# lcicek/Critic-VAE

Hardware: AMD Instinct MI355X
Metric: VAE train-step images/sec on 64x64x3 frames (higher is better)
Workload: dtype f32

## Files before the change

critic-vae_amd/csrc/api.hip:

```cpp
#include "common.h"
#include "../../include/cvae.h"
#include <stdarg.h>
#include <stdio.h>
#include <stdlib.h>
#include <string.h>
#include <cmath>
#include <string>
#include <vector>

static thread_local char g_err[512] = "";
void cvae_set_error(const char* fmt, ...) {
    va_list ap;
    va_start(ap, fmt);
    vsnprintf(g_err, sizeof(g_err), fmt, ap);
    va_end(ap);
}

static constexpr int PROBE_IDS = 32, PROBE_CAP = 128;
struct ProbeSlot { hipEvent_t e0[PROBE_CAP], e1[PROBE_CAP]; int n = 0; bool made = false; };
struct ProbeState { uint32_t mask = 0; ProbeSlot slot[PROBE_IDS]; };
static thread_local ProbeSlot* g_probe_cur = nullptr;
void cvae_probe_begin(hipStream_t st) {
    ProbeSlot* p = g_probe_cur;
    if (p && p->n < PROBE_CAP) (void)hipEventRecord(p->e0[p->n], st);
// ... 22 lines not shown
}

int persistent_grid(int wgs_per_cu, int num_items) {
    static const int maxwg = [] { const char* e = getenv("CVAE_PERSIST_MAXWG"); const int n = e ? atoi(e) : 0; return n > 0 ? n : 0; }();
    int G = wgs_per_cu * cvae_num_cus();
    if (maxwg > 0 && G > maxwg) G = maxwg;
    G -= G % 8;
    if (G < 8) G = 8;
    return G < num_items ? G : num_items;
}
extern "C" int32_t cvae_conv_route(int32_t precision, int32_t width, int32_t layer, int32_t dgrad, int64_t batch) {
    if ((width != 64 && width != 128) || layer < 0 || layer > 3 || precision < 0 || precision > 3 || batch < 1 || batch > 0x7fffffffLL) return CVAE_EINVAL;
    if (layer == 0 && (precision != 1 || dgrad != 0)) return CVAE_EINVAL;
    return conv_route(precision, layer, width, dgrad != 0, batch).family;
}

struct ParamEntry { std::string name; int64_t offset, numel; };

struct WsLayout {
    int64_t y[4], a[4], coef[4], bnpart[4];
    int64_t zcat, h, o[4];
    int64_t dout4, d_o[4], d_h, d_zcat, d_a[4], d_y[4];
    int64_t wc[3];
    int64_t xp;
    int64_t wpack;
    int64_t ms, scratch_w, scratch, total;
};

struct cvae_handle_s {
    cvae_config cfg;
    std::vector<ParamEntry> params;
    int64_t param_total;
    int K;
    int enc_w[4], enc_b[4], enc_g[4], enc_be[4], fc_w, fc_b, dec_w[5], dec_b[5], di_w, di_b;
    hipStream_t side = nullptr;
    hipEvent_t ev_ready[8] = {}, ev_side = nullptr;
    bool streams_ready = false;
    const void* xp_ws = nullptr;
    int xp_B = 0;
    struct { int pass = 0, next = 0, B = 0; const void* ws = nullptr; const double* rec = nullptr; } sync;
    ProbeState probe;
};

struct ProbeArm {
    ProbeArm(cvae_handle_s* h, int kind, int layer) {
        const int id = kind * 9 + layer;
// ... 23 lines not shown
    auto take = [&](int64_t n) { int64_t o = off; off += align_up(n, 64); return o; };
    const bool b16 = h->cfg.precision == 1;
    auto act = [&](int64_t elems) { return take(b16 ? (elems + 1) / 2 : elems); };
    for (int l = 0; l < 4; ++l) {
        const int64_t H = layer_h(h, l), C = kLayers[l].cout;
        w.y[l] = act(B * H * H * C);
        w.a[l] = act(B * (H / 2) * (H / 2) * C);
        w.coef[l] = take(C * 4);
        w.bnpart[l] = take((int64_t)2 * bn_num_tiles(l, W, B) * C);
        w.d_y[l] = l == 0 ? -1 : act(B * H * H * C);
        w.d_a[l] = act(B * (H / 2) * (H / 2) * C);
    }
    w.zcat = take((int64_t)B * 33);
    w.d_zcat = take((int64_t)B * 33);
    w.h = act((int64_t)B * h->K);
    w.d_h = act((int64_t)B * h->K);
    for (int i = 0; i < 4; ++i) {
        const int64_t H = layer_h(h, 4 + i), C = kLayers[4 + i].cout;
        w.o[i] = act(B * H * H * C);
        w.d_o[i] = act(B * H * H * C);
    }
    w.dout4 = take(b16 ? 0 : (int64_t)B * 3 * W * W);
    for (int i = 0; i < 3; ++i) w.wc[i] = take(conv_up_wc_floats(5 + i));
    w.xp = take(b16 ? (int64_t)B * W * W * 2 : 0);
    w.wpack = take(h->cfg.precision != 0 ? conv_bf16_pack_floats(h->cfg.precision >= 2 ? 3 : 1) : 0);
    w.ms = take(msssim_ws_floats(W, B));
    int64_t sc = 0, scw = 0;
    auto mx = [&](int64_t v) { if (v > sc) sc = v; };
    for (int l = 1; l <= 4; ++l) { if (wgrad_ws_floats(l, W, B) > scw) scw = wgrad_ws_floats(l, W, B);
        if (h->cfg.precision == 1 && conv_bf16_supported(l, W) && wgrad_bf16_ws_floats(l, W, B) > scw) scw = wgrad_bf16_ws_floats(l, W, B);
        if (h->cfg.precision >= 2 && conv_bf16_supported(l, W) && wgrad_split_ws_floats(l, W, B) > scw) scw = wgrad_split_ws_floats(l, W, B);
        mx(conv_fwd_ws_floats(l, W, B)); mx(conv_dgrad_ws_floats(l, W, B)); }
    for (int l = 5; l <= 7; ++l) { if (conv_up_wgrad_ws_floats(l, W, B) > scw) scw = conv_up_wgrad_ws_floats(l, W, B); mx(conv_up_ws_floats(l, W, B)); }
    if (e1_wgrad_ws_floats(W, B) > scw) scw = e1_wgrad_ws_floats(W, B);
    w.scratch_w = take(scw);
    mx(scw + 36 * 128 * 64);
    mx(d4_bwd_ws_floats(W, B));
    for (int l = 0; l < 4; ++l) { mx(bn_bwd_ws_floats(l, W, B)); mx(bn_fwd_ws_floats(l, W)); }
    mx(fc_ws_floats(W, B));
    mx(colsum_ws_floats(0, 256));
    w.scratch = take(sc);
    w.total = off;
    return w;
}

static void add_param(cvae_handle_s* h, int* idx, const char* name, int64_t numel) {
// ... 43 lines not shown
    }
    delete h;
}

int64_t cvae_param_total(cvae_handle h) { return h->param_total; }
int32_t cvae_param_count(cvae_handle h) { return (int32_t)h->params.size(); }
const char* cvae_param_name(cvae_handle h, int32_t i) { return h->params[i].name.c_str(); }
int64_t cvae_param_offset(cvae_handle h, int32_t i) { return h->params[i].offset; }
int64_t cvae_param_numel(cvae_handle h, int32_t i) { return h->params[i].numel; }
int64_t cvae_workspace_bytes(cvae_handle h, int32_t batch) { return carve(h, batch).total * 4; }
int64_t cvae_bn_state_floats(cvae_handle) { return 2 * 480; }

int64_t cvae_ws_offset(cvae_handle h, int32_t batch, const char* name) {
    const WsLayout w = carve(h, batch);
    char nm[32];
    for (int l = 0; l < 4; ++l) {
        snprintf(nm, sizeof nm, "y%d", l); if (!strcmp(name, nm)) return w.y[l];
        snprintf(nm, sizeof nm, "a%d", l); if (!strcmp(name, nm)) return w.a[l];
        snprintf(nm, sizeof nm, "d_y%d", l); if (!strcmp(name, nm)) return w.d_y[l];
        snprintf(nm, sizeof nm, "d_a%d", l); if (!strcmp(name, nm)) return w.d_a[l];
        snprintf(nm, sizeof nm, "coef%d", l); if (!strcmp(name, nm)) return w.coef[l];
        snprintf(nm, sizeof nm, "o%d", l); if (!strcmp(name, nm)) return w.o[l];
        snprintf(nm, sizeof nm, "d_o%d", l); if (!strcmp(name, nm)) return w.d_o[l];
    }
    if (!strcmp(name, "zcat")) return w.zcat;
    if (!strcmp(name, "d_zcat")) return w.d_zcat;
    if (!strcmp(name, "h")) return w.h;
    if (!strcmp(name, "d_h")) return w.d_h;
    if (!strcmp(name, "dout4")) return w.dout4;
    if (!strcmp(name, "scratch")) return w.scratch;
    if (!strcmp(name, "ms")) return w.ms;
    if (!strcmp(name, "xp")) return h->cfg.precision == 1 ? w.xp : -1;
    return -1;
}

static const int kBnOff[4] = {0, 32, 96, 224};
static const int64_t kSyncOff[9] = {0, 97, 289, 673, 1441, 1452, 1964, 2220, 2348};
static const int64_t kSyncCnt[9] = {97, 192, 384, 768, 11, 512, 256, 128, 64};
static const int64_t kSyncCount = 96;
static_assert(2348 + 64 == CVAE_SYNC_DOUBLES, "sync record size");
int cvae_decode(cvae_handle h, int32_t B, const float* zcat, const float* params, float* recon, void* wsv, void* stream);
int cvae_backward_phases(cvae_handle h, int32_t B, const float* x, const float* pred, const float* eps, const float* params,
                         const float* logvar, const float* recon, const float* d_recon, const float* d_mu,
                         const float* d_logvar, void* wsv, float* grads, int32_t phase_mask, void* stream);

#define P_(idx) (params + h->params[(idx)].offset)
// ... 228 lines not shown
        return 0;
    }
    int join() {
        if (!overlap) return 0;
        HIPRC(hipEventRecord(h->ev_side, h->side));
        HIPRC(hipStreamWaitEvent(st, h->ev_side, 0));
        return 0;
    }
    int decoder() {
        { ProbeArm pa(h, 1, 8);
          RC(launch_d4_bwd(W, B, ws + w.o[3], d_recon, recon, P_(h->dec_w[4]), ws + w.dout4, ws + w.d_o[3],
                           G_(h->dec_w[4]), G_(h->dec_b[4]), sc, st, io_bf16(h))); }
        for (int i = 3; i >= 0; --i) {
            const int l = 4 + i;
            const float* in = i == 0 ? ws + w.h : ws + w.o[i - 1];
            RC(fork(3 - i));
            if (i == 0) {
                { ProbeArm pa(h, 2, l); RC(conv_wgrad(h, 4, B, in, ws + w.d_o[0], G_(h->dec_w[0]), G_(h->dec_b[0]), scw, sd)); }
                { ProbeArm pa(h, 1, l);
                  if (use_bf16(h, 4)) RC(launch_conv_dgrad_bf16(4, W, bf16_mode(h), B, ws + w.d_o[0], ws + w.wpack, ws + w.d_h, ws + w.scratch, st));
                  else RC(launch_conv_dgrad(l, W, B, ws + w.d_o[0], P_(h->dec_w[0]), nullptr, ws + w.d_h, ws + w.scratch, st)); }
            } else {
                { ProbeArm pa(h, 2, l);
                  RC(launch_conv_up_wgrad(l, W, B, in, ws + w.d_o[i], G_(h->dec_w[i]), G_(h->dec_b[i]), scw, sd, use_bf16_wgrad(h, l))); }
                { ProbeArm pa(h, 1, l);
                  if (use_bf16(h, l)) RC(launch_conv_up_dgrad_bf16(l, W, bf16_mode(h), B, ws + w.d_o[i], ws + w.wpack, ws + w.o[i - 1], ws + w.d_o[i - 1], st));
                  else RC(launch_conv_up_dgrad(l, W, B, ws + w.d_o[i], ws + w.wc[i - 1], ws + w.o[i - 1], ws + w.d_o[i - 1], sc, st)); }
            }
        }
        RC(launch_decin_bwd(W, B, ws + w.zcat, ws + w.d_h, P_(h->di_w), G_(h->di_w), G_(h->di_b), ws + w.d_zcat, sc, st, io_bf16(h)));
        return join();
    }
    int fc() {
        return launch_fc_bwd(W, B, ws + w.a[3], P_(h->fc_w), ws + w.d_zcat, eps, logvar, d_mu, d_logvar, G_(h->fc_w),
                             G_(h->fc_b), ws + w.d_a[3], sc, st, io_bf16(h));
    }
    int bn(int l, int stage, double* rec, const double* count) {
        ProbeArm pa(h, 3, l);
        return launch_bn_pool_act_bwd(l, W, B, ws + w.y[l], ws + w.a[l], ws + w.d_a[l], ws + w.coef[l], P_(h->enc_g[l]),
                                      l == 0 ? nullptr : ws + w.d_y[l], G_(h->enc_g[l]), G_(h->enc_be[l]), nullptr, sc, st, io_bf16(h),
                                      stage, rec, count);
    }
    int block_grads(int l) {
        RC(fork(7 - l));
        if (l == 0) {
            const float* fu[7] = {ws + w.y[0], ws + w.a[0], ws + w.d_a[0], ws + w.coef[0], bn_bwd_bcoef(0, W, B, sc),
                                  P_(h->enc_w[0]), P_(h->enc_b[0])};
// ... 818 lines not shown
```

critic-vae_amd/csrc/bn.hip:

```cpp
#include "common.h"

struct BnGeom { int C, H, act; };
static inline BnGeom bn_geom(int layer, int width) {
    const int s = width / 64;
    return BnGeom{kLayers[layer].cout, kLayers[layer].h * s, layer == 3 ? 1 : 0};
}
static inline void part_geom(int layer, int H, int* imgs, int* pxPerImg, int* tilesPerImg) {
    if (layer == 0) { *imgs = 1; *pxPerImg = 512; *tilesPerImg = (H / 16) * (H / 32); return; }
    const TileGeom t = tile_geom(H);
    *imgs = t.IMGS; *pxPerImg = t.PX_PER_IMG; *tilesPerImg = t.TILES_PER_IMG;
}
int bn_num_tiles(int layer, int width, int B) {
    const BnGeom g = bn_geom(layer, width);
    int imgs, ppi, tpi;
    part_geom(layer, g.H, &imgs, &ppi, &tpi);
    return cdiv(B, imgs) * tpi;
}

__global__ __launch_bounds__(256) void bn_fwd_reduce_kernel(const float* __restrict__ part, int numTiles, int C, int B,
                                                            int imgsPerTile, int pxPerImg, int tilesPerImg,
                                                            double* __restrict__ mid, int tilesPerBlk) {
    __shared__ double red[3][8][32];
    const int cl = threadIdx.x & 31, rg = threadIdx.x >> 5, c = blockIdx.x * 32 + cl;
    const int t0 = blockIdx.y * tilesPerBlk;
    int t1 = t0 + tilesPerBlk; if (t1 > numTiles) t1 = numTiles;
    double S = 0.0, Q = 0.0, M = 0.0;
#pragma unroll 4
    for (int t = t0 + rg; t < t1; t += 8) {
        const int img0 = (t / tilesPerImg) * imgsPerTile;
        int ni = B - img0; if (ni > imgsPerTile) ni = imgsPerTile;
        const double n = (double)(ni * pxPerImg);
        const double s = (double)part[(size_t)t * C + c];
        S += s; Q += s * s / n; M += (double)part[((size_t)numTiles + t) * C + c];
    }
    red[0][rg][cl] = S; red[1][rg][cl] = Q; red[2][rg][cl] = M;
    __syncthreads();
    if (rg == 0) {
        for (int k = 1; k < 8; ++k) { S += red[0][k][cl]; Q += red[1][k][cl]; M += red[2][k][cl]; }
        double* o = mid + (size_t)blockIdx.y * 3 * C;
        o[c] = S; o[C + c] = Q; o[2 * C + c] = M;
    }
}

__device__ __forceinline__ void bn_fwd_coef(int c, double S, double Q, double M, double N, const float* __restrict__ gamma,
                                            const float* __restrict__ beta, float* __restrict__ run_mean,
                                            float* __restrict__ run_var, float* __restrict__ coef, int train) {
    float mean, var;
    if (train) {
        const double mu = S / N;
        double v = (M + Q - S * S / N) / N;
        if (v < 0.0) v = 0.0;
        mean = (float)mu; var = (float)v;
        const float uvar = (float)(v * N / (N - 1.0));
        {
#pragma clang fp contract(off)
            run_mean[c] = 0.9f * run_mean[c] + 0.1f * mean;
            run_var[c] = 0.9f * run_var[c] + 0.1f * uvar;
        }
    } else {
        mean = run_mean[c]; var = run_var[c];
    }
    const float invstd = 1.0f / sqrtf(var + 1e-5f);
    const float scale = gamma[c] * invstd;
    coef[c * 4 + 0] = scale;
    coef[c * 4 + 1] = beta[c] - mean * scale;
    coef[c * 4 + 2] = mean;
    coef[c * 4 + 3] = invstd;
}

struct BnSums { double S, Q, M; };
__device__ __forceinline__ BnSums bn_fwd_merge(const double* __restrict__ mid, int RA, int C, int c, int r) {
    BnSums s{0.0, 0.0, 0.0};
    if (r < RA) { s.S = mid[(size_t)r * 3 * C + c]; s.Q = mid[(size_t)r * 3 * C + C + c]; s.M = mid[(size_t)r * 3 * C + 2 * C + c]; }
#pragma unroll
    for (int o = 16; o > 0; o >>= 1) { s.S += __shfl_xor(s.S, o, 64); s.Q += __shfl_xor(s.Q, o, 64); s.M += __shfl_xor(s.M, o, 64); }
    return s;
}

__global__ __launch_bounds__(64) void bn_fwd_finalize_kernel(const double* __restrict__ mid, int RA, int C, double N,
                                                             const float* __restrict__ gamma, const float* __restrict__ beta,
                                                             float* __restrict__ run_mean, float* __restrict__ run_var,
                                                             float* __restrict__ coef, int train) {
    const int c = blockIdx.x * 2 + (threadIdx.x >> 5), r = threadIdx.x & 31;
    const BnSums s = bn_fwd_merge(mid, train ? RA : 0, C, c, r);
    if (r != 0) return;
    bn_fwd_coef(c, s.S, s.Q, s.M, N, gamma, beta, run_mean, run_var, coef, train);
}

__global__ __launch_bounds__(64) void bn_fwd_record_kernel(const double* __restrict__ mid, int RA, int C, double* __restrict__ rec,
                                                           double* __restrict__ count, double images) {
    const int c = blockIdx.x * 2 + (threadIdx.x >> 5), r = threadIdx.x & 31;
    const BnSums s = bn_fwd_merge(mid, RA, C, c, r);
    if (r != 0) return;
    rec[c] = s.S; rec[C + c] = s.Q; rec[2 * C + c] = s.M;
    if (count && c == 0) *count = images;
}

__global__ __launch_bounds__(64) void bn_fwd_finish_kernel(const double* __restrict__ rec, const double* __restrict__ count, int C, int H,
                                                           const float* __restrict__ gamma, const float* __restrict__ beta,
                                                           float* __restrict__ run_mean, float* __restrict__ run_var,
                                                           float* __restrict__ coef) {
    const int c = blockIdx.x * 64 + threadIdx.x;
    if (c >= C) return;
    const double N = count[0] * H * H;
    bn_fwd_coef(c, rec[c], rec[C + c], rec[2 * C + c], N, gamma, beta, run_mean, run_var, coef, 1);
}

__device__ __forceinline__ float act_fwd(float v, int act) { return act ? tanhf(v) : fmaxf(v, 0.f); }
__device__ __forceinline__ float act_bwd_from_out(float a, int act) { return act ? (1.f - a * a) : (a > 0.f ? 1.f : 0.f); }
// ... 168 lines not shown
#pragma unroll
                for (int p = 0; p < 4; ++p) yy[p] = A::ld(y, base + window_px(p, H, C) + c);
                int pos;
                const float ym = window_argmax(yy, coef[c * 4], coef[c * 4 + 1], &pos);
                s2[e] += ((float)av[e] > 0.f ? (float)gv[e] : 0.f) * ((ym - coef[c * 4 + 2]) * coef[c * 4 + 3]);
            }
        }
    }
#pragma unroll
    for (int e = 0; e < V; ++e) { red[0][threadIdx.x][e] = s1[e]; red[1][threadIdx.x][e] = s2[e]; }
    __syncthreads();
    if (sub == 0) {
        for (int k = 1; k < NSUB; ++k)
#pragma unroll
            for (int e = 0; e < V; ++e) { s1[e] += red[0][k * CV + cv][e]; s2[e] += red[1][k * CV + cv][e]; }
#pragma unroll
        for (int e = 0; e < V; ++e) {
            part[((size_t)blockIdx.x * 2) * C + cv * V + e] = s1[e];
            part[((size_t)blockIdx.x * 2 + 1) * C + cv * V + e] = s2[e];
        }
    }
}

template <bool REC>
__global__ __launch_bounds__(256) void bn_bwd_finalize_kernel(const float* __restrict__ rows, int R, int64_t stride, int C, float invN,
                                                              float* __restrict__ dgamma, float* __restrict__ dbeta, float* __restrict__ bcoef,
                                                              double* __restrict__ rec) {
    const int c = blockIdx.x * 16 + (threadIdx.x >> 4), q = threadIdx.x & 15;
    float s1 = 0.f, s2 = 0.f;
    if (c < C)
        for (int r = q; r < R; r += 16) { s1 += rows[(size_t)r * stride + c]; s2 += rows[(size_t)r * stride + C + c]; }
#pragma unroll
    for (int o = 8; o > 0; o >>= 1) { s1 += __shfl_xor(s1, o, 64); s2 += __shfl_xor(s2, o, 64); }
    if (c < C && q == 0) {
        dgamma[c] = s2; dbeta[c] = s1;
        if (REC) { rec[c] = (double)s1; rec[C + c] = (double)s2; }
        else { bcoef[c * 2] = s1 * invN; bcoef[c * 2 + 1] = s2 * invN; }
    }
}

__global__ __launch_bounds__(256) void bn_bwd_finish_kernel(const double* __restrict__ rec, const double* __restrict__ count, int C, int H,
                                                            float* __restrict__ bcoef) {
    const int c = blockIdx.x * 256 + threadIdx.x;
    if (c >= C) return;
    const float invN = (float)(1.0 / (double)(float)(count[0] * H * H));
    bcoef[c * 2] = (float)rec[c] * invN;
    bcoef[c * 2 + 1] = (float)rec[C + c] * invN;
}

static constexpr int BN_RA = 32;
int64_t bn_fwd_ws_floats(int layer, int width) { (void)width; return (int64_t)2 * BN_RA * 3 * kLayers[layer].cout; }

static int bn_fwd_reduce(int layer, int width, int B, const float* bnpart, float* ws, hipStream_t st, int tilesPerPartial, int* RA_out) {
    const BnGeom g = bn_geom(layer, width);
    int imgs, ppi, tpi;
    part_geom(layer, g.H, &imgs, &ppi, &tpi);
    int numTiles = cdiv(B, imgs) * tpi;
    if (tilesPerPartial > 1) {
        const int T = tilesPerPartial;
        numTiles = cdiv(numTiles, T);
        if (tpi >= T) { ppi *= T; tpi /= T; }
        else if (tpi > 1) { imgs = T / tpi; ppi *= tpi; tpi = 1; }
        else imgs *= T;
    }
    double* mid = reinterpret_cast<double*>(ws);
    const int tpb = cdiv(numTiles, BN_RA);
    const int RA = cdiv(numTiles, tpb);
    hipLaunchKernelGGL(bn_fwd_reduce_kernel, dim3(g.C / 32, RA), dim3(256), 0, st, bnpart, numTiles, g.C, B, imgs,
                       ppi, tpi, mid, tpb);
    CVAE_CHECK_LAUNCH();
    *RA_out = RA;
    return 0;
}

int launch_bn_fwd_finalize(int layer, int width, int B, const float* bnpart, const float* gamma, const float* beta,
                           float* run_mean, float* run_var, float* coef, float* ws, int train, hipStream_t st, int tilesPerPartial) {
    const BnGeom g = bn_geom(layer, width);
    double* mid = reinterpret_cast<double*>(ws);
    int RA = 0;
    if (train) { int rc = bn_fwd_reduce(layer, width, B, bnpart, ws, st, tilesPerPartial, &RA); if (rc) return rc; }
    hipLaunchKernelGGL(bn_fwd_finalize_kernel, dim3(g.C / 2), dim3(64), 0, st, mid, RA, g.C,
                       (double)B * g.H * g.H, gamma, beta, run_mean, run_var, coef, train);
    CVAE_CHECK_LAUNCH();
    return 0;
}

int launch_bn_fwd_record(int layer, int width, int B, const float* bnpart, float* ws, hipStream_t st, int tilesPerPartial,
                         double* rec, double* count) {
    const BnGeom g = bn_geom(layer, width);
    int RA = 0;
    { int rc = bn_fwd_reduce(layer, width, B, bnpart, ws, st, tilesPerPartial, &RA); if (rc) return rc; }
    hipLaunchKernelGGL(bn_fwd_record_kernel, dim3(g.C / 2), dim3(64), 0, st, reinterpret_cast<const double*>(ws), RA, g.C,
                       rec, count, (double)B);
    CVAE_CHECK_LAUNCH();
    return 0;
}

int launch_bn_fwd_finish(int layer, int width, const double* rec, const double* count, const float* gamma, const float* beta,
                         float* run_mean, float* run_var, float* coef, hipStream_t st) {
    const BnGeom g = bn_geom(layer, width);
    hipLaunchKernelGGL(bn_fwd_finish_kernel, dim3(cdiv(g.C, 64)), dim3(64), 0, st, rec, count, g.C, g.H, gamma, beta,
                       run_mean, run_var, coef);
    CVAE_CHECK_LAUNCH();
    return 0;
}
// ... 37 lines not shown
static BnBwdKernels bn_bwd_kernels() {
    if constexpr (ACT == 0) return {bn_bwd_stats_relu_kernel<AT>, bn_bwd_kernel<AT, 0, 1>};
    else return {bn_bwd_kernel<AT, ACT, 0>, bn_bwd_kernel<AT, ACT, 1>};
}

int launch_bn_pool_act_bwd(int layer, int width, int B, const float* y, const float* a, const float* da,
                           const float* coef, const float* gamma, float* dy, float* dgamma, float* dbeta,
                           float* dbias, float* ws, hipStream_t st, bool bf16io, int stage, double* rec, const double* count) {
    (void)gamma;
    const BnGeom g = bn_geom(layer, width);
    const int64_t totalPx = (int64_t)B * (g.H / 2) * (g.H / 2);
    const int nblk = bn_bwd_blocks(totalPx, g.C);
    const int64_t ppb = (totalPx + nblk - 1) / nblk;
    float* part = ws;
    float* bcoef = ws + (size_t)nblk * 2 * g.C;
    float* red = bcoef + 2 * g.C;
    float* crws = red + 2 * g.C;
    const float invN = 1.0f / (float)((double)B * g.H * g.H);
    const BnBwdKernels k = bf16io ? (g.act ? bn_bwd_kernels<__bf16, 1>() : bn_bwd_kernels<__bf16, 0>())
                                  : (g.act ? bn_bwd_kernels<float, 1>() : bn_bwd_kernels<float, 0>());
    if (stage != 2) {
        hipLaunchKernelGGL(k.stats, dim3(nblk), dim3(256), 0, st, y, a, da, coef, nullptr, nullptr, part, g.C, g.H, totalPx, ppb);
        CVAE_CHECK_LAUNCH();
        const float* rows; int R; int64_t rstride;
        { int rc = launch_col_reduce_partial(part, nblk, 2 * g.C, 2 * g.C, crws, st, &rows, &R, &rstride); if (rc) return rc; }
        if (stage == 1) hipLaunchKernelGGL(bn_bwd_finalize_kernel<true>, dim3(cdiv(g.C, 16)), dim3(256), 0, st, rows, R, rstride, g.C, invN, dgamma, dbeta, nullptr, rec);
        else hipLaunchKernelGGL(bn_bwd_finalize_kernel<false>, dim3(cdiv(g.C, 16)), dim3(256), 0, st, rows, R, rstride, g.C, invN, dgamma, dbeta, bcoef, nullptr);
        CVAE_CHECK_LAUNCH();
        if (stage == 1) return 0;
    } else {
        hipLaunchKernelGGL(bn_bwd_finish_kernel, dim3(cdiv(g.C, 256)), dim3(256), 0, st, rec, count, g.C, g.H, bcoef);
        CVAE_CHECK_LAUNCH();
    }
    if (!dy) {
        if (dbias) { cvae_set_error("bn_bwd: dbias needs the apply pass (dy)"); return -2; }
        return 0;
    }
    cvae_probe_begin(st);
    hipLaunchKernelGGL(k.apply, dim3(nblk), dim3(256), 0, st, y, a, da, coef, bcoef, dy, part, g.C, g.H, totalPx, ppb);
    cvae_probe_end(st);
    CVAE_CHECK_LAUNCH();
    if (dbias) return launch_col_reduce(part, nblk, g.C, g.C, dbias, crws, st);
    return 0;
}
```

critic-vae_amd/csrc/common.h:

```cpp
#pragma once
#include <hip/hip_runtime.h>
#include <stdint.h>
#include <stddef.h>
#include <atomic>

typedef float f32x16 __attribute__((ext_vector_type(16)));
typedef float f32x4 __attribute__((ext_vector_type(4)));
typedef __bf16 bf16x8 __attribute__((ext_vector_type(8)));

typedef __bf16 bf16x4 __attribute__((ext_vector_type(4)));

template <typename AT> struct Act;
template <> struct Act<float> {
    static constexpr bool BF16 = false;
    static __device__ __forceinline__ float ld(const float* p, size_t i) { return p[i]; }
    static __device__ __forceinline__ void st(float* p, size_t i, float v) { p[i] = v; }
    static __device__ __forceinline__ f32x4 ld4(const float* p, size_t i) { return *reinterpret_cast<const f32x4*>(p + i); }
    static __device__ __forceinline__ void st4(float* p, size_t i, f32x4 v) { *reinterpret_cast<f32x4*>(p + i) = v; }
    template <int V> using Vec = float __attribute__((ext_vector_type(V)));
    template <int V> static __device__ __forceinline__ Vec<V> ldv(const float* p, size_t i) {
        static_assert(V == 1 || V == 4, "fp32 storage: scalar or float4 accesses");
        return *reinterpret_cast<const Vec<V>*>(p + i);
    }
    template <int V> static __device__ __forceinline__ void stv(float* p, size_t i, Vec<V> v) {
// ... 191 lines not shown
                  float* xp = nullptr);
int launch_e1_wgrad(int width, int B, const float* x, const float* dy, float* dw, float* dbias, float* ws,
                    hipStream_t st, bool bf16 = false, const float* const* fuse = nullptr,
                    const float* xp = nullptr);
const float* bn_bwd_bcoef(int layer, int width, int B, const float* ws);
int64_t e1_wgrad_ws_floats(int width, int B);
int launch_d4_fwd(int width, int B, const float* in, const float* w, const float* bias, float* recon,
                  hipStream_t st, bool bf16io = false);
int64_t d4_bwd_ws_floats(int width, int B);
int launch_d4_bwd(int width, int B, const float* o3, const float* d_recon, const float* recon,
                  const float* w, float* dout, float* d_o3, float* dw, float* db, float* ws,
                  hipStream_t st, bool bf16io = false);
int64_t conv_up_wc_floats(int layer);
int launch_collapse_w(int layer, const float* w, float* wc, hipStream_t st);
int launch_collapse_w3(const float* const w[3], float* const wc[3], hipStream_t st);
int64_t conv_up_ws_floats(int layer, int width, int B);
int launch_conv_up_fwd(int layer, int width, int B, const float* in, const float* wc, const float* bias,
                       float* out, float* ws, hipStream_t st);
int launch_conv_up_dgrad(int layer, int width, int B, const float* dout, const float* wc, const float* aux,
                         float* din, float* ws, hipStream_t st);
int64_t conv_up_wgrad_ws_floats(int layer, int width, int B);
int launch_conv_up_wgrad(int layer, int width, int B, const float* in, const float* dout, float* dw,
                         float* dbias, float* ws, hipStream_t st, bool bf16 = false);
int launch_up_wgrad_bf16_main(int layer, int width, int B, const float* in, const float* dout, float* slab, int Smax, int* S_out, hipStream_t st,
                              int* plan = nullptr);
int conv_wgrad_bf16_plan(int layer, int width, int B, int plan[3]);
int conv_up_wgrad_bf16_plan(int layer, int width, int B, int plan[3]);
int bn_num_tiles(int layer, int width, int B);
int launch_bn_fwd_finalize(int layer, int width, int B, const float* bnpart, const float* gamma,
                           const float* beta, float* run_mean, float* run_var, float* coef,
                           float* ws, int train, hipStream_t st, int tilesPerPartial = 1);
int launch_bn_fwd_record(int layer, int width, int B, const float* bnpart, float* ws, hipStream_t st, int tilesPerPartial,
                         double* rec, double* count);
int launch_bn_fwd_finish(int layer, int width, const double* rec, const double* count, const float* gamma, const float* beta,
                         float* run_mean, float* run_var, float* coef, hipStream_t st);
int64_t bn_fwd_ws_floats(int layer, int width);
int launch_bn_pool_act_fwd(int layer, int width, int B, const float* y, const float* coef, float* a,
                           hipStream_t st, bool bf16io = false);
int64_t bn_bwd_ws_floats(int layer, int width, int B);
int launch_bn_pool_act_bwd(int layer, int width, int B, const float* y, const float* a,
                           const float* da, const float* coef, const float* gamma, float* dy,
                           float* dgamma, float* dbeta, float* dbias, float* ws, hipStream_t st, bool bf16io = false,
                           int stage = 0, double* rec = nullptr, const double* count = nullptr);
struct LatentPlan {
    int fc_fwd_gemm;
    int di_imgs, di_blocks;
// ... 116 lines not shown
```

critic-vae_amd/csrc/conv_up.hip:

```cpp
#include "common.h"

static constexpr int KC = 16, KCP = 17;

template <int HS>
struct UpTile {
    static constexpr int TW = HS < 32 ? HS : 32;
    static constexpr int TH = (128 / TW) < HS ? (128 / TW) : HS;
    static constexpr int IMGS = 128 / (TW * TH);
    static constexpr int HTW = TW + 2, HTH = TH + 2, HPI = HTW * HTH, HP = IMGS * HPI;
    static constexpr int PS = ((HP + 5) / 8) * 8 + 2;
    static constexpr int TILES_X = HS / TW, TILES_Y = HS / TH, TILES_PER_IMG = TILES_X * TILES_Y;
};

__device__ __forceinline__ int phase_lo(int ph, int a) { return ph == 0 ? (a == 0 ? 0 : a == 1 ? 2 : 4) : (a == 0 ? 0 : a == 1 ? 1 : 3); }
__device__ __forceinline__ int phase_hi(int ph, int a) { return ph == 0 ? (a == 0 ? 1 : a == 1 ? 3 : 4) : (a == 0 ? 0 : a == 1 ? 2 : 4); }
__device__ __forceinline__ int phase_of(int ph, int r) { return ph == 0 ? (r >> 1) : ((r + 1) >> 1); }

struct CollapseJobs { const float* w[3]; float* wc[3]; int n[3]; };
__global__ __launch_bounds__(256) void collapse_w_kernel(CollapseJobs jobs) {
    const float* __restrict__ w = jobs.w[blockIdx.z];
    float* __restrict__ wc = jobs.wc[blockIdx.z];
    const int n = jobs.n[blockIdx.z];
    const int i = blockIdx.x * 256 + threadIdx.x;
    if (i >= n) return;
    const int t = blockIdx.y, p = t / 9, a = (t % 9) / 3, b = t % 3, py = p >> 1, px = p & 1;
    float acc = 0.f;
    for (int r = phase_lo(py, a); r <= phase_hi(py, a); ++r)
        for (int s = phase_lo(px, b); s <= phase_hi(px, b); ++s) acc += w[(size_t)(r * 5 + s) * n + i];
    wc[(size_t)t * n + i] = acc;
}

__global__ __launch_bounds__(256) void expand_dw_kernel(const float* __restrict__ rows, int R, int64_t stride,
                                                        float* __restrict__ dw, int n, float* __restrict__ dbias,
                                                        int cout) {
    const int i = blockIdx.x * 256 + threadIdx.x;
    if (dbias != nullptr && blockIdx.x == 0 && blockIdx.y == 0 && (int)threadIdx.x < cout) {
        float b = 0.f;
        for (int q = 0; q < R; ++q) b += rows[(size_t)q * stride + (size_t)36 * n + threadIdx.x];
        dbias[threadIdx.x] = b;
    }
    if (i >= n) return;
    const int r = blockIdx.y / 5, s = blockIdx.y % 5;
    float acc = 0.f;
#pragma unroll
    for (int p = 0; p < 4; ++p) {
        const float* src = rows + (size_t)(p * 9 + phase_of(p >> 1, r) * 3 + phase_of(p & 1, s)) * n + i;
        float a = 0.f;
        for (int q = 0; q < R; ++q) a += src[(size_t)q * stride];
        acc += a;
    }
    dw[(size_t)blockIdx.y * n + i] = acc;
}

struct UpArgs {
    const float* in;
    const float* wc;
    const float* bias;
// ... 455 lines not shown

int launch_conv_up_dgrad(int layer, int width, int B, const float* dout, const float* wc, const float* aux, float* din,
                         float* ws, hipStream_t st) {
    if (width == 64) {
        switch (layer) {
            case 5: return run_up_dgrad<128, 64, 4, 64, UP_KS5>(B, dout, wc, aux, din, ws, st);
            case 6: return run_up_dgrad<64, 32, 8, 64, UP_KS6>(B, dout, wc, aux, din, ws, st);
            case 7: return run_up_dgrad<32, 32, 16, 32, 1>(B, dout, wc, aux, din, ws, st);
        }
    }
    if (width == 128) {
        switch (layer) {
            case 5: return run_up_dgrad<128, 64, 8, 64, UP_KS5>(B, dout, wc, aux, din, ws, st);
            case 6: return run_up_dgrad<64, 32, 16, 64, UP_KS6>(B, dout, wc, aux, din, ws, st);
            case 7: return run_up_dgrad<32, 32, 32, 32, 1>(B, dout, wc, aux, din, ws, st);
        }
    }
    cvae_set_error("conv_up_dgrad: unsupported layer %d at width %d", layer, width);
    return -2;
}

template <int CIN, int COUT, int HS>
static int run_up_wgrad(int B, const float* in, const float* dout, float* dw, float* dbias, float* ws, hipStream_t st,
                        int64_t* need, int bf16_layer = 0, int bf16_width = 64, int* plan = nullptr) {
    using T = UpTile64<HS>;
    const int numTiles = cdiv(B, T::IMGS) * T::TILES_PER_IMG;
    const int bps = (CIN / 32) * (COUT / 32);
    const int cus = cvae_num_cus();
    int Scap = cdiv(2 * cus, bps);
    if (Scap > numTiles) Scap = numTiles;
    int S = cdiv(cus, bps);
    if (S > numTiles) S = numTiles;
    const int tps = cdiv(numTiles, S);
    S = cdiv(numTiles, tps);
    const int64_t nc = (int64_t)36 * CIN * COUT, row = nc + COUT;
    if (plan) return launch_up_wgrad_bf16_main(bf16_layer, bf16_width, B, nullptr, nullptr, nullptr, Scap, &S, st, plan);
    if (need) { *need = (int64_t)(Scap + 17) * row; return 0; }
    if (bf16_layer) {
        int rc = launch_up_wgrad_bf16_main(bf16_layer, bf16_width, B, in, dout, ws, Scap, &S, st);
        if (rc) return rc;
    } else {
        UpWgradArgs a{in, dout, ws, B, numTiles, tps};
        cvae_probe_begin(st);
        hipLaunchKernelGGL((conv_up_wgrad_kernel<CIN, COUT, HS>), dim3(S, CIN / 32, COUT / 32), dim3(256), 0, st, a);
        cvae_probe_end(st);
        CVAE_CHECK_LAUNCH();
    }
    float* mid = ws + (size_t)S * row;
    float* red = mid + (size_t)16 * row;
    { int rc = launch_reduce_slabs(ws, red, row, S, row, st, mid); if (rc) return rc; }
    const float* rows = red;
    const int R = 1;
    static_assert(COUT <= 256, "expand_dw_kernel sums the bias gradient in one workgroup");
    hipLaunchKernelGGL(expand_dw_kernel, dim3(cdiv(CIN * COUT, 256), 25), dim3(256), 0, st, rows, R, row, dw, CIN * COUT, dbias, COUT);
    CVAE_CHECK_LAUNCH();
    return 0;
}

static int dispatch_up_wgrad(int layer, int width, int B, const float* in, const float* dout, float* dw, float* dbias,
                             float* ws, hipStream_t st, int64_t* need, bool bf16 = false, int* plan = nullptr) {
    if (width == 64) {
        switch (layer) {
            case 5: return run_up_wgrad<128, 64, 4>(B, in, dout, dw, dbias, ws, st, need, bf16 ? 5 : 0, 64, plan);
            case 6: return run_up_wgrad<64, 32, 8>(B, in, dout, dw, dbias, ws, st, need, bf16 ? 6 : 0, 64, plan);
            case 7: return run_up_wgrad<32, 32, 16>(B, in, dout, dw, dbias, ws, st, need, bf16 ? 7 : 0, 64, plan);
        }
    }
    if (width == 128) {
        switch (layer) {
            case 5: return run_up_wgrad<128, 64, 8>(B, in, dout, dw, dbias, ws, st, need, bf16 ? 5 : 0, 128, plan);
            case 6: return run_up_wgrad<64, 32, 16>(B, in, dout, dw, dbias, ws, st, need, bf16 ? 6 : 0, 128, plan);
            case 7: return run_up_wgrad<32, 32, 32>(B, in, dout, dw, dbias, ws, st, need, bf16 ? 7 : 0, 128, plan);
        }
    }
    cvae_set_error("conv_up_wgrad: unsupported layer %d at width %d", layer, width);
    return -2;
}
int64_t conv_up_wgrad_ws_floats(int layer, int width, int B) {
    int64_t need = 0;
    if (dispatch_up_wgrad(layer, width, B, nullptr, nullptr, nullptr, nullptr, nullptr, nullptr, &need)) return 0;
    return need;
}
int conv_up_wgrad_bf16_plan(int layer, int width, int B, int plan[3]) {
    return dispatch_up_wgrad(layer, width, B, nullptr, nullptr, nullptr, nullptr, nullptr, nullptr, nullptr, true, plan);
}
int launch_conv_up_wgrad(int layer, int width, int B, const float* in, const float* dout, float* dw, float* dbias,
                         float* ws, hipStream_t st, bool bf16) {
    return dispatch_up_wgrad(layer, width, B, in, dout, dw, dbias, ws, st, nullptr, bf16);
}
```

Baseline: 90490.

## Batch decoder expand_dw launches and fuse BN reduce/finalize into single kernels

Decoder up-conv wgrad now writes its reduced slab into dedicated workspace buffers, and one batched expand_dw launch covers all three layers, replacing three separate launches. BN forward statistics use a single 1024-thread kernel that reduces and finalizes when the tile count is small. BN backward in stage 0 skips the column-reduce pass and finalizes directly from the partials. The aim is to cut kernel launches and intermediate passes in a launch-bound train step. The cost is extra workspace and a batched expand that now runs only after the last wgrad has finished.

```diff
diff --git a/critic-vae_amd/csrc/api.hip b/critic-vae_amd/csrc/api.hip
--- a/critic-vae_amd/csrc/api.hip
+++ b/critic-vae_amd/csrc/api.hip
@@ -68,6 +68,7 @@
     int64_t zcat, h, o[4];
     int64_t dout4, d_o[4], d_h, d_zcat, d_a[4], d_y[4];
     int64_t wc[3];
+    int64_t up_red[3];
     int64_t xp;
     int64_t wpack;
     int64_t ms, scratch_w, scratch, total;
@@ -137,6 +138,7 @@
     }
     w.dout4 = take(b16 ? 0 : (int64_t)B * 3 * W * W);
     for (int i = 0; i < 3; ++i) w.wc[i] = take(conv_up_wc_floats(5 + i));
+    for (int i = 0; i < 3; ++i) w.up_red[i] = take(conv_up_red_floats(5 + i));
     w.xp = take(b16 ? (int64_t)B * W * W * 2 : 0);
     w.wpack = take(h->cfg.precision != 0 ? conv_bf16_pack_floats(h->cfg.precision >= 2 ? 3 : 1) : 0);
     w.ms = take(msssim_ws_floats(W, B));
@@ -226,6 +228,7 @@
         snprintf(nm, sizeof nm, "coef%d", l); if (!strcmp(name, nm)) return w.coef[l];
         snprintf(nm, sizeof nm, "o%d", l); if (!strcmp(name, nm)) return w.o[l];
         snprintf(nm, sizeof nm, "d_o%d", l); if (!strcmp(name, nm)) return w.d_o[l];
+        snprintf(nm, sizeof nm, "up_red%d", l); if (l < 3 && !strcmp(name, nm)) return w.up_red[l];
     }
     if (!strcmp(name, "zcat")) return w.zcat;
     if (!strcmp(name, "d_zcat")) return w.d_zcat;
@@ -500,7 +503,13 @@
                   else RC(launch_conv_dgrad(l, W, B, ws + w.d_o[0], P_(h->dec_w[0]), nullptr, ws + w.d_h, ws + w.scratch, st)); }
             } else {
                 { ProbeArm pa(h, 2, l);
-                  RC(launch_conv_up_wgrad(l, W, B, in, ws + w.d_o[i], G_(h->dec_w[i]), G_(h->dec_b[i]), scw, sd, use_bf16_wgrad(h, l))); }
+                  RC(launch_conv_up_wgrad_reduce(l, W, B, in, ws + w.d_o[i], ws + w.up_red[i - 1], scw, sd, use_bf16_wgrad(h, l))); }
+                if (i == 1) {
+                    const float* red[3] = {ws + w.up_red[0], ws + w.up_red[1], ws + w.up_red[2]};
+                    float* dw[3] = {G_(h->dec_w[1]), G_(h->dec_w[2]), G_(h->dec_w[3])};
+                    float* db[3] = {G_(h->dec_b[1]), G_(h->dec_b[2]), G_(h->dec_b[3])};
+                    RC(launch_expand_dw3(red, dw, db, sd));
+                }
                 { ProbeArm pa(h, 1, l);
                   if (use_bf16(h, l)) RC(launch_conv_up_dgrad_bf16(l, W, bf16_mode(h), B, ws + w.d_o[i], ws + w.wpack, ws + w.o[i - 1], ws + w.d_o[i - 1], st));
                   else RC(launch_conv_up_dgrad(l, W, B, ws + w.d_o[i], ws + w.wc[i - 1], ws + w.o[i - 1], ws + w.d_o[i - 1], sc, st)); }
diff --git a/critic-vae_amd/csrc/bn.hip b/critic-vae_amd/csrc/bn.hip
--- a/critic-vae_amd/csrc/bn.hip
+++ b/critic-vae_amd/csrc/bn.hip
@@ -15,6 +15,21 @@
     int imgs, ppi, tpi;
     part_geom(layer, g.H, &imgs, &ppi, &tpi);
     return cdiv(B, imgs) * tpi;
+}
+
+struct BnSums { double S, Q, M; };
+__device__ __forceinline__ BnSums bn_fwd_rows(const float* __restrict__ part, int numTiles, int C, int B, int imgsPerTile, int pxPerImg,
+                                              int tilesPerImg, int c, int t0, int t1, int rg) {
+    BnSums a{0.0, 0.0, 0.0};
+#pragma unroll 4
+    for (int t = t0 + rg; t < t1; t += 8) {
+        const int img0 = (t / tilesPerImg) * imgsPerTile;
+        int ni = B - img0; if (ni > imgsPerTile) ni = imgsPerTile;
+        const double n = (double)(ni * pxPerImg);
+        const double s = (double)part[(size_t)t * C + c];
+        a.S += s; a.Q += s * s / n; a.M += (double)part[((size_t)numTiles + t) * C + c];
+    }
+    return a;
 }
 
 __global__ __launch_bounds__(256) void bn_fwd_reduce_kernel(const float* __restrict__ part, int numTiles, int C, int B,
@@ -24,15 +39,8 @@
     const int cl = threadIdx.x & 31, rg = threadIdx.x >> 5, c = blockIdx.x * 32 + cl;
     const int t0 = blockIdx.y * tilesPerBlk;
     int t1 = t0 + tilesPerBlk; if (t1 > numTiles) t1 = numTiles;
-    double S = 0.0, Q = 0.0, M = 0.0;
-#pragma unroll 4
-    for (int t = t0 + rg; t < t1; t += 8) {
-        const int img0 = (t / tilesPerImg) * imgsPerTile;
-        int ni = B - img0; if (ni > imgsPerTile) ni = imgsPerTile;
-        const double n = (double)(ni * pxPerImg);
-        const double s = (double)part[(size_t)t * C + c];
-        S += s; Q += s * s / n; M += (double)part[((size_t)numTiles + t) * C + c];
-    }
+    const BnSums a = bn_fwd_rows(part, numTiles, C, B, imgsPerTile, pxPerImg, tilesPerImg, c, t0, t1, rg);
+    double S = a.S, Q = a.Q, M = a.M;
     red[0][rg][cl] = S; red[1][rg][cl] = Q; red[2][rg][cl] = M;
     __syncthreads();
     if (rg == 0) {
@@ -68,7 +76,6 @@
     coef[c * 4 + 3] = invstd;
 }
 
-struct BnSums { double S, Q, M; };
 __device__ __forceinline__ BnSums bn_fwd_merge(const double* __restrict__ mid, int RA, int C, int c, int r) {
     BnSums s{0.0, 0.0, 0.0};
     if (r < RA) { s.S = mid[(size_t)r * 3 * C + c]; s.Q = mid[(size_t)r * 3 * C + C + c]; s.M = mid[(size_t)r * 3 * C + 2 * C + c]; }
@@ -85,6 +92,30 @@
     const BnSums s = bn_fwd_merge(mid, train ? RA : 0, C, c, r);
     if (r != 0) return;
     bn_fwd_coef(c, s.S, s.Q, s.M, N, gamma, beta, run_mean, run_var, coef, train);
+}
+
+__global__ __launch_bounds__(1024) void bn_fwd_stats_kernel(const float* __restrict__ part, int numTiles, int C, int B,
+                                                            int imgsPerTile, int pxPerImg, int tilesPerImg, int tilesPerBlk, int RA,
+                                                            double N, const float* __restrict__ gamma, const float* __restrict__ beta,
+                                                            float* __restrict__ run_mean, float* __restrict__ run_var,
+                                                            float* __restrict__ coef) {
+    __shared__ double red[32][3][8][4];
+    const int cl = threadIdx.x & 3, rg = (threadIdx.x >> 2) & 7, ra = threadIdx.x >> 5;
+    const int t0 = ra * tilesPerBlk;
+    int t1 = t0 + tilesPerBlk; if (t1 > numTiles) t1 = numTiles;
+    BnSums a = bn_fwd_rows(part, numTiles, C, B, imgsPerTile, pxPerImg, tilesPerImg, blockIdx.x * 4 + cl, t0, t1, rg);
+    red[ra][0][rg][cl] = a.S; red[ra][1][rg][cl] = a.Q; red[ra][2][rg][cl] = a.M;
+    __syncthreads();
+    if (rg == 0) {
+        for (int k = 1; k < 8; ++k) { a.S += red[ra][0][k][cl]; a.Q += red[ra][1][k][cl]; a.M += red[ra][2][k][cl]; }
+        red[ra][0][0][cl] = a.S; red[ra][1][0][cl] = a.Q; red[ra][2][0][cl] = a.M;
+    }
+    __syncthreads();
+    if (threadIdx.x >= 128) return;
+    const int cm = threadIdx.x >> 5, r = threadIdx.x & 31;
+    const BnSums s = bn_fwd_merge(&red[0][0][0][0], RA, 32, cm, r);
+    if (r != 0) return;
+    bn_fwd_coef(blockIdx.x * 4 + cm, s.S, s.Q, s.M, N, gamma, beta, run_mean, run_var, coef, 1);
 }
 
 __global__ __launch_bounds__(64) void bn_fwd_record_kernel(const double* __restrict__ mid, int RA, int C, double* __restrict__ rec,
@@ -299,20 +330,54 @@
     }
 }
 
+struct BnBwdSums { float s1, s2; };
+__device__ __forceinline__ BnBwdSums bn_bwd_merge(const float* __restrict__ rows, int R, int64_t stride, int C, int c, int q, bool live) {
+    float s1 = 0.f, s2 = 0.f;
+    if (live)
+        for (int r = q; r < R; r += 16) { s1 += rows[(size_t)r * stride + c]; s2 += rows[(size_t)r * stride + C + c]; }
+#pragma unroll
+    for (int o = 8; o > 0; o >>= 1) { s1 += __shfl_xor(s1, o, 64); s2 += __shfl_xor(s2, o, 64); }
+    return BnBwdSums{s1, s2};
+}
+
 template <bool REC>
 __global__ __launch_bounds__(256) void bn_bwd_finalize_kernel(const float* __restrict__ rows, int R, int64_t stride, int C, float invN,
                                                               float* __restrict__ dgamma, float* __restrict__ dbeta, float* __restrict__ bcoef,
                                                               double* __restrict__ rec) {
     const int c = blockIdx.x * 16 + (threadIdx.x >> 4), q = threadIdx.x & 15;
-    float s1 = 0.f, s2 = 0.f;
-    if (c < C)
-        for (int r = q; r < R; r += 16) { s1 += rows[(size_t)r * stride + c]; s2 += rows[(size_t)r * stride + C + c]; }
-#pragma unroll
-    for (int o = 8; o > 0; o >>= 1) { s1 += __shfl_xor(s1, o, 64); s2 += __shfl_xor(s2, o, 64); }
+    const BnBwdSums s = bn_bwd_merge(rows, R, stride, C, c, q, c < C);
     if (c < C && q == 0) {
-        dgamma[c] = s2; dbeta[c] = s1;
-        if (REC) { rec[c] = (double)s1; rec[C + c] = (double)s2; }
-        else { bcoef[c * 2] = s1 * invN; bcoef[c * 2 + 1] = s2 * invN; }
+        dgamma[c] = s.s2; dbeta[c] = s.s1;
+        if (REC) { rec[c] = (double)s.s1; rec[C + c] = (double)s.s2; }
+        else { bcoef[c * 2] = s.s1 * invN; bcoef[c * 2 + 1] = s.s2 * invN; }
+    }
+}
+
+__global__ __launch_bounds__(1024) void bn_bwd_rows_finalize_kernel(const float* __restrict__ part, int R, int C, int rowsPerBlk, float invN,
+                                                                    float* __restrict__ dgamma, float* __restrict__ dbeta,
+                                                                    float* __restrict__ bcoef) {
+    __shared__ float red[32][2][8][4];
+    const int cl = threadIdx.x & 3, rl = (threadIdx.x >> 2) & 7, ra = threadIdx.x >> 5, c = blockIdx.x * 4 + cl;
+    const int r0 = ra * rowsPerBlk;
+    int r1 = r0 + rowsPerBlk; if (r1 > R) r1 = R;
+    float a1 = 0.f, a2 = 0.f;
+#pragma unroll 4
+    for (int r = r0 + rl; r < r1; r += 8) { a1 += part[(size_t)r * 2 * C + c]; a2 += part[(size_t)r * 2 * C + C + c]; }
+    red[ra][0][rl][cl] = a1; red[ra][1][rl][cl] = a2;
+    __syncthreads();
+    if (rl == 0) {
+#pragma unroll
+        for (int k = 1; k < 8; ++k) { a1 += red[ra][0][k][cl]; a2 += red[ra][1][k][cl]; }
+        red[ra][0][0][cl] = a1; red[ra][1][0][cl] = a2;
+    }
+    __syncthreads();
+    if (threadIdx.x >= 64) return;
+    const int cm = threadIdx.x >> 4, q = threadIdx.x & 15;
+    const BnBwdSums s = bn_bwd_merge(&red[0][0][0][0], cdiv(R, rowsPerBlk), 64, 32, cm, q, true);
+    if (q == 0) {
+        const int co = blockIdx.x * 4 + cm;
+        dgamma[co] = s.s2; dbeta[co] = s.s1;
+        bcoef[co * 2] = s.s1 * invN; bcoef[co * 2 + 1] = s.s2 * invN;
     }
 }
 
@@ -328,7 +393,8 @@
 static constexpr int BN_RA = 32;
 int64_t bn_fwd_ws_floats(int layer, int width) { (void)width; return (int64_t)2 * BN_RA * 3 * kLayers[layer].cout; }
 
-static int bn_fwd_reduce(int layer, int width, int B, const float* bnpart, float* ws, hipStream_t st, int tilesPerPartial, int* RA_out) {
+struct BnFwdPlan { int numTiles, imgs, ppi, tpi, tpb, RA; };
+static BnFwdPlan bn_fwd_plan(int layer, int width, int B, int tilesPerPartial) {
     const BnGeom g = bn_geom(layer, width);
     int imgs, ppi, tpi;
     part_geom(layer, g.H, &imgs, &ppi, &tpi);
@@ -340,24 +406,38 @@
         else if (tpi > 1) { imgs = T / tpi; ppi *= tpi; tpi = 1; }
         else imgs *= T;
     }
+    const int tpb = cdiv(numTiles, BN_RA);
+    return BnFwdPlan{numTiles, imgs, ppi, tpi, tpb, cdiv(numTiles, tpb)};
+}
+
+static int bn_fwd_reduce(int layer, int width, int B, const float* bnpart, float* ws, hipStream_t st, int tilesPerPartial, int* RA_out) {
+    const BnGeom g = bn_geom(layer, width);
+    const BnFwdPlan p = bn_fwd_plan(layer, width, B, tilesPerPartial);
     double* mid = reinterpret_cast<double*>(ws);
-    const int tpb = cdiv(numTiles, BN_RA);
-    const int RA = cdiv(numTiles, tpb);
-    hipLaunchKernelGGL(bn_fwd_reduce_kernel, dim3(g.C / 32, RA), dim3(256), 0, st, bnpart, numTiles, g.C, B, imgs,
-                       ppi, tpi, mid, tpb);
+    hipLaunchKernelGGL(bn_fwd_reduce_kernel, dim3(g.C / 32, p.RA), dim3(256), 0, st, bnpart, p.numTiles, g.C, B, p.imgs,
+                       p.ppi, p.tpi, mid, p.tpb);
     CVAE_CHECK_LAUNCH();
-    *RA_out = RA;
+    *RA_out = p.RA;
     return 0;
 }
+
+static constexpr int BN_FWD_ONE_LAUNCH_TILES = 512;
 
 int launch_bn_fwd_finalize(int layer, int width, int B, const float* bnpart, const float* gamma, const float* beta,
                            float* run_mean, float* run_var, float* coef, float* ws, int train, hipStream_t st, int tilesPerPartial) {
     const BnGeom g = bn_geom(layer, width);
-    double* mid = reinterpret_cast<double*>(ws);
+    const double N = (double)B * g.H * g.H;
+    const BnFwdPlan p = bn_fwd_plan(layer, width, B, tilesPerPartial);
+    if (train && p.numTiles <= BN_FWD_ONE_LAUNCH_TILES) {
+        hipLaunchKernelGGL(bn_fwd_stats_kernel, dim3(g.C / 4), dim3(1024), 0, st, bnpart, p.numTiles, g.C, B, p.imgs, p.ppi, p.tpi,
+                           p.tpb, p.RA, N, gamma, beta, run_mean, run_var, coef);
+        CVAE_CHECK_LAUNCH();
+        return 0;
+    }
     int RA = 0;
     if (train) { int rc = bn_fwd_reduce(layer, width, B, bnpart, ws, st, tilesPerPartial, &RA); if (rc) return rc; }
-    hipLaunchKernelGGL(bn_fwd_finalize_kernel, dim3(g.C / 2), dim3(64), 0, st, mid, RA, g.C,
-                       (double)B * g.H * g.H, gamma, beta, run_mean, run_var, coef, train);
+    hipLaunchKernelGGL(bn_fwd_finalize_kernel, dim3(g.C / 2), dim3(64), 0, st, reinterpret_cast<const double*>(ws), RA, g.C,
+                       N, gamma, beta, run_mean, run_var, coef, train);
     CVAE_CHECK_LAUNCH();
     return 0;
 }
@@ -441,10 +521,15 @@
     if (stage != 2) {
         hipLaunchKernelGGL(k.stats, dim3(nblk), dim3(256), 0, st, y, a, da, coef, nullptr, nullptr, part, g.C, g.H, totalPx, ppb);
         CVAE_CHECK_LAUNCH();
-        const float* rows; int R; int64_t rstride;
-        { int rc = launch_col_reduce_partial(part, nblk, 2 * g.C, 2 * g.C, crws, st, &rows, &R, &rstride); if (rc) return rc; }
-        if (stage == 1) hipLaunchKernelGGL(bn_bwd_finalize_kernel<true>, dim3(cdiv(g.C, 16)), dim3(256), 0, st, rows, R, rstride, g.C, invN, dgamma, dbeta, nullptr, rec);
-        else hipLaunchKernelGGL(bn_bwd_finalize_kernel<false>, dim3(cdiv(g.C, 16)), dim3(256), 0, st, rows, R, rstride, g.C, invN, dgamma, dbeta, bcoef, nullptr);
+        if (stage == 1) {
+            const float* rows; int R; int64_t rstride;
+            { int rc = launch_col_reduce_partial(part, nblk, 2 * g.C, 2 * g.C, crws, st, &rows, &R, &rstride); if (rc) return rc; }
+            hipLaunchKernelGGL(bn_bwd_finalize_kernel<true>, dim3(cdiv(g.C, 16)), dim3(256), 0, st, rows, R, rstride, g.C, invN, dgamma, dbeta, nullptr, rec);
+        } else if (nblk > 64) {
+            hipLaunchKernelGGL(bn_bwd_rows_finalize_kernel, dim3(g.C / 4), dim3(1024), 0, st, part, nblk, g.C, cdiv(nblk, 32), invN, dgamma, dbeta, bcoef);
+        } else {
+            hipLaunchKernelGGL(bn_bwd_finalize_kernel<false>, dim3(cdiv(g.C, 16)), dim3(256), 0, st, part, nblk, (int64_t)2 * g.C, g.C, invN, dgamma, dbeta, bcoef, nullptr);
+        }
         CVAE_CHECK_LAUNCH();
         if (stage == 1) return 0;
     } else {
diff --git a/critic-vae_amd/csrc/common.h b/critic-vae_amd/csrc/common.h
--- a/critic-vae_amd/csrc/common.h
+++ b/critic-vae_amd/csrc/common.h
@@ -237,6 +237,10 @@
 int64_t conv_up_wgrad_ws_floats(int layer, int width, int B);
 int launch_conv_up_wgrad(int layer, int width, int B, const float* in, const float* dout, float* dw,
                          float* dbias, float* ws, hipStream_t st, bool bf16 = false);
+int64_t conv_up_red_floats(int layer);
+int launch_conv_up_wgrad_reduce(int layer, int width, int B, const float* in, const float* dout, float* red, float* ws, hipStream_t st,
+                                bool bf16 = false);
+int launch_expand_dw3(const float* const red[3], float* const dw[3], float* const dbias[3], hipStream_t st);
 int launch_up_wgrad_bf16_main(int layer, int width, int B, const float* in, const float* dout, float* slab, int Smax, int* S_out, hipStream_t st,
                               int* plan = nullptr);
 int conv_wgrad_bf16_plan(int layer, int width, int B, int plan[3]);
diff --git a/critic-vae_amd/csrc/conv_up.hip b/critic-vae_amd/csrc/conv_up.hip
--- a/critic-vae_amd/csrc/conv_up.hip
+++ b/critic-vae_amd/csrc/conv_up.hip
@@ -30,9 +30,13 @@
     wc[(size_t)t * n + i] = acc;
 }
 
-__global__ __launch_bounds__(256) void expand_dw_kernel(const float* __restrict__ rows, int R, int64_t stride,
-                                                        float* __restrict__ dw, int n, float* __restrict__ dbias,
-                                                        int cout) {
+struct ExpandJobs { const float* rows[3]; float* dw[3]; float* dbias[3]; int R[3]; int64_t stride[3]; int n[3]; int cout[3]; };
+__global__ __launch_bounds__(256) void expand_dw_kernel(ExpandJobs jobs) {
+    const float* __restrict__ rows = jobs.rows[blockIdx.z];
+    float* __restrict__ dw = jobs.dw[blockIdx.z];
+    float* __restrict__ dbias = jobs.dbias[blockIdx.z];
+    const int R = jobs.R[blockIdx.z], n = jobs.n[blockIdx.z], cout = jobs.cout[blockIdx.z];
+    const int64_t stride = jobs.stride[blockIdx.z];
     const int i = blockIdx.x * 256 + threadIdx.x;
     if (dbias != nullptr && blockIdx.x == 0 && blockIdx.y == 0 && (int)threadIdx.x < cout) {
         float b = 0.f;
@@ -534,7 +538,7 @@
 
 template <int CIN, int COUT, int HS>
 static int run_up_wgrad(int B, const float* in, const float* dout, float* dw, float* dbias, float* ws, hipStream_t st,
-                        int64_t* need, int bf16_layer = 0, int bf16_width = 64, int* plan = nullptr) {
+                        int64_t* need, int bf16_layer = 0, int bf16_width = 64, int* plan = nullptr, float* red_out = nullptr) {
     using T = UpTile64<HS>;
     const int numTiles = cdiv(B, T::IMGS) * T::TILES_PER_IMG;
     const int bps = (CIN / 32) * (COUT / 32);
@@ -559,30 +563,30 @@
         CVAE_CHECK_LAUNCH();
     }
     float* mid = ws + (size_t)S * row;
-    float* red = mid + (size_t)16 * row;
+    float* red = red_out ? red_out : mid + (size_t)16 * row;
     { int rc = launch_reduce_slabs(ws, red, row, S, row, st, mid); if (rc) return rc; }
-    const float* rows = red;
-    const int R = 1;
+    if (red_out) return 0;
     static_assert(COUT <= 256, "expand_dw_kernel sums the bias gradient in one workgroup");
-    hipLaunchKernelGGL(expand_dw_kernel, dim3(cdiv(CIN * COUT, 256), 25), dim3(256), 0, st, rows, R, row, dw, CIN * COUT, dbias, COUT);
+    ExpandJobs jobs{{red, nullptr, nullptr}, {dw, nullptr, nullptr}, {dbias, nullptr, nullptr}, {1, 0, 0}, {row, 0, 0}, {CIN * COUT, 0, 0}, {COUT, 0, 0}};
+    hipLaunchKernelGGL(expand_dw_kernel, dim3(cdiv(CIN * COUT, 256), 25, 1), dim3(256), 0, st, jobs);
     CVAE_CHECK_LAUNCH();
     return 0;
 }
 
 static int dispatch_up_wgrad(int layer, int width, int B, const float* in, const float* dout, float* dw, float* dbias,
-                             float* ws, hipStream_t st, int64_t* need, bool bf16 = false, int* plan = nullptr) {
+                             float* ws, hipStream_t st, int64_t* need, bool bf16 = false, int* plan = nullptr, float* red_out = nullptr) {
     if (width == 64) {
         switch (layer) {
-            case 5: return run_up_wgrad<128, 64, 4>(B, in, dout, dw, dbias, ws, st, need, bf16 ? 5 : 0, 64, plan);
-            case 6: return run_up_wgrad<64, 32, 8>(B, in, dout, dw, dbias, ws, st, need, bf16 ? 6 : 0, 64, plan);
-            case 7: return run_up_wgrad<32, 32, 16>(B, in, dout, dw, dbias, ws, st, need, bf16 ? 7 : 0, 64, plan);
+            case 5: return run_up_wgrad<128, 64, 4>(B, in, dout, dw, dbias, ws, st, need, bf16 ? 5 : 0, 64, plan, red_out);
+            case 6: return run_up_wgrad<64, 32, 8>(B, in, dout, dw, dbias, ws, st, need, bf16 ? 6 : 0, 64, plan, red_out);
+            case 7: return run_up_wgrad<32, 32, 16>(B, in, dout, dw, dbias, ws, st, need, bf16 ? 7 : 0, 64, plan, red_out);
         }
     }
     if (width == 128) {
         switch (layer) {
-            case 5: return run_up_wgrad<128, 64, 8>(B, in, dout, dw, dbias, ws, st, need, bf16 ? 5 : 0, 128, plan);
-            case 6: return run_up_wgrad<64, 32, 16>(B, in, dout, dw, dbias, ws, st, need, bf16 ? 6 : 0, 128, plan);
-            case 7: return run_up_wgrad<32, 32, 32>(B, in, dout, dw, dbias, ws, st, need, bf16 ? 7 : 0, 128, plan);
+            case 5: return run_up_wgrad<128, 64, 8>(B, in, dout, dw, dbias, ws, st, need, bf16 ? 5 : 0, 128, plan, red_out);
+            case 6: return run_up_wgrad<64, 32, 16>(B, in, dout, dw, dbias, ws, st, need, bf16 ? 6 : 0, 128, plan, red_out);
+            case 7: return run_up_wgrad<32, 32, 32>(B, in, dout, dw, dbias, ws, st, need, bf16 ? 7 : 0, 128, plan, red_out);
         }
     }
     cvae_set_error("conv_up_wgrad: unsupported layer %d at width %d", layer, width);
@@ -600,3 +604,21 @@
                          float* ws, hipStream_t st, bool bf16) {
     return dispatch_up_wgrad(layer, width, B, in, dout, dw, dbias, ws, st, nullptr, bf16);
 }
+int64_t conv_up_red_floats(int layer) { return conv_up_wc_floats(layer) + kLayers[layer].cout; }
+int launch_conv_up_wgrad_reduce(int layer, int width, int B, const float* in, const float* dout, float* red, float* ws, hipStream_t st,
+                                bool bf16) {
+    return dispatch_up_wgrad(layer, width, B, in, dout, nullptr, nullptr, ws, st, nullptr, bf16, nullptr, red);
+}
+int launch_expand_dw3(const float* const red[3], float* const dw[3], float* const dbias[3], hipStream_t st) {
+    ExpandJobs jobs;
+    int nmax = 0;
+    for (int i = 0; i < 3; ++i) {
+        const int n = kLayers[5 + i].cin * kLayers[5 + i].cout;
+        jobs.rows[i] = red[i]; jobs.dw[i] = dw[i]; jobs.dbias[i] = dbias[i];
+        jobs.R[i] = 1; jobs.stride[i] = conv_up_red_floats(5 + i); jobs.n[i] = n; jobs.cout[i] = kLayers[5 + i].cout;
+        if (n > nmax) nmax = n;
+    }
+    hipLaunchKernelGGL(expand_dw_kernel, dim3(cdiv(nmax, 256), 25, 3), dim3(256), 0, st, jobs);
+    CVAE_CHECK_LAUNCH();
+    return 0;
+}
```

New measurement: 90430. No clear change (-0.1%).
